# OpenDataPlane/odp

Hardware: AMD Instinct MI355X
Metric: Mpkts/s classified device-resident (higher is better)
Workload: dtype u8; 1 GPU; config3; packets_per_gpu=1000000, packets_total=1000000, rules=256, cos=33, frame_bytes=IMIX 60/566/1514 7:4:1, streams=1, rotate=4, parallelism=shard1

## Files before the change

odp_amd/csrc/mi_cls.hip:

```cpp
#include "mi_cls_dev.h"

#include "mi_cls_asm.h"
#include "mi_cls_spec.h"

#include <errno.h>
#include <unistd.h>

#include <algorithm>
#include <array>
#include <map>
#include <memory>
#include <mutex>
#include <set>
#include <string>
#include <thread>
#include <vector>

struct mi_cls_ctx {
	int device;
	uint32_t *d_dev;
	size_t dev_cap;
	int loaded;
	MiProgram prog;
	int wpb;
// ... 290 lines not shown
	const bool small = (long)hot_bytes <= (long)hot_max;
	const bool full4 = small && 4 * (st_of(4) + hot_bytes) <= LDS_CU;
	const bool small_batch = c->batch_hint != 0 &&
				 c->batch_hint < 2u * (uint32_t)c->num_cu * 16u * WAVE;
	int nw = 4;
	bool lt = full4;
	for (int w : { 16, 12, 8 })
		if (st_of(w) + hot_bytes <= LDS_CU) {
			nw = w;
			lt = true;
			break;
		}
	if ((nw == 8 || small_batch) && full4) {
		nw = 4;
		lt = true;
	}
	if (wpb_env == 4 || wpb_env == 8 || wpb_env == 12 || wpb_env == 16) {
		nw = wpb_env;
		lt = nw == 4 ? small && st_of(4) + hot_bytes <= LDS_CU : st_of(nw) + hot_bytes <= LDS_CU;
		if (nw != 4 && nw != 16 && !lt)
			nw = 16;
	}
	if (opt != 0 && nw != 4) {
		nw = 16;
		lt = st_of(16) + hot_bytes <= LDS_CU;
		if (!lt)
			nw = 4;
	}
	const size_t lds_block = st_of(nw) + (lt ? hot_bytes : 0);
	int per_cu = (int)(LDS_CU / lds_block);
	const int occ = MIN_WAVES_PER_EU;
	if (per_cu > occ * 4 / nw)
		per_cu = occ * 4 / nw;
	if (per_cu_env > 0)
		per_cu = per_cu_env;
	if (per_cu < 1)
		per_cu = 1;
	return Shape{ nw, lt, lt ? hot_bytes : 0, per_cu };
}


static void dump_spec(const std::string &src)
{
	const char *dp = getenv("MI_CLS_DUMP_SPEC");
	FILE *f = dp ? fopen(dp, "w") : nullptr;
	if (f) {
		fputs(src.c_str(), f);
		fclose(f);
	}
}

extern "C" int mi_cls_spec_compile(const void *tbl, size_t bytes, int nw)
{
	MiProgram p;
	const int rc = mi_asm_compile(tbl, bytes, mi_asm_knobs_from_env(), p);
	if (rc)
		return rc;
	if (nw != 4 && nw != 12 && nw != 16)
		return -EINVAL;
	if (p.spec_mode < 0 && p.plan.empty())
		return 1;
	std::string inst;
	const std::string src = mi_asm_spec_program(p, nw, true, false, inst);
	dump_spec(src);
	return mi_spec_compile_now(src, inst);
}

static bool spec_enabled(void)
{
	const char *e = getenv("MI_CLS_JIT");
	return !(e && e[0] == '0');
}

static void spec_setup(mi_cls_ctx_t *c)
{
	c->spec.reset();
	c->spec_fn = nullptr;
	const bool ck = c->opt != 0;
	const bool flat = c->prog.spec_mode >= 0;
	if ((!flat && c->prog.plan.empty()) || !spec_enabled())
		return;
	const Shape sh = pick_shape(c, c->opt);
	if (ck ? ((flat && !sh.lt) || (sh.nw != 4 && sh.nw != 16))
	       : flat ? (!sh.lt || (sh.nw != 4 && sh.nw != 12 && sh.nw != 16))
		      : (sh.nw != 4 && sh.nw != 8 && sh.nw != 12 && sh.nw != 16))
		return;
	std::string inst;
	const std::string src = mi_asm_spec_program(c->prog, sh.nw, flat ? true : sh.lt, ck, inst);
	dump_spec(src);
	c->spec = mi_spec_request(src, inst);
	c->spec_nw = sh.nw;
	c->spec_lt = sh.lt;
	c->spec_ck = ck;
}

static hipFunction_t spec_fn(mi_cls_ctx_t *c, bool wait)
{
	if (c->spec_fn || !c->spec)
		return c->spec_fn;
	hipFunction_t fn = nullptr;
	if (!mi_spec_function(*c->spec, c->device, wait, &fn))
		return nullptr;
	if (!fn)
		c->spec.reset();
	c->spec_fn = fn;
	return fn;
}


extern "C" int mi_cls_last_launch(const mi_cls_ctx_t *c, uint32_t *info, uint32_t n)
{
	if (!c || (!info && n))
		return -EINVAL;
	const uint32_t k = n < MI_CLS_LAUNCH_INFO_WORDS ? n : MI_CLS_LAUNCH_INFO_WORDS;
	memcpy(info, c->last, k * sizeof(uint32_t));
	return (int)k;
}

extern "C" int mi_cls_spec_wait(mi_cls_ctx_t *c)
{
	if (!c || !c->loaded)
		return -EINVAL;
	if (!c->spec)
		return 1;
	return spec_fn(c, true) ? 0 : 1;
}

extern "C" int mi_cls_classify(mi_cls_ctx_t *c, const uint8_t *pkts, const uint32_t *off,
			       const uint16_t *len, uint32_t n, mi_cls_result_t *out, void *stream)
{
	if (!c || !c->loaded)
		return -EINVAL;
	if (n == 0)
		return 0;
	if (!pkts || !off || !len || !out)
		return -EINVAL;
	if (((uintptr_t)out & 15u) != 0)
		return -EINVAL;
	HIP_OK(hipSetDevice(c->device));
	KArgs a;
	a.pkts = pkts;
	a.off = off;
	a.len = len;
	a.n = n;
	a.dev = c->d_dev;
	a.out = out;
	a.stats = c->stats_on ? c->d_stats : nullptr;
	a.opt = c->opt;
	a.hint = c->d_hint;
	a.seq = ++c->seq;
	if (a.seq == 0u)
		a.seq = c->seq = 2u;
	memcpy(a.stats_mask, c->stats_mask, sizeof(a.stats_mask));
	const Shape sh = pick_shape(c, c->opt);
	const int nw = sh.nw;
	const bool lt = sh.lt;
	const bool div = c->prog.tree;
	const uint32_t bthreads = (uint32_t)nw * WAVE;
	uint32_t tiles = (n + bthreads - 1) / bthreads;
	uint32_t max_grid = (uint32_t)c->num_cu * (uint32_t)sh.per_cu;
	uint32_t grid = tiles < max_grid ? tiles : max_grid;
	const size_t dyn = sh.dyn;
	hipStream_t st = (hipStream_t)stream;
	int lrc;
	uint32_t *last = c->last;
	last[0] = (uint32_t)nw;
	last[1] = lt;
	last[2] = 0;
	last[3] = 0;
	last[4] = 0;
	last[5] = c->opt != 0;
	last[6] = grid;
	const bool spec_ok = c->spec && c->spec_ck == (c->opt != 0) && c->spec_nw == nw &&
			     c->spec_lt == lt && spec_fn(c, false);
	if (c->opt != 0 && spec_ok) {
		last[2] = c->prog.flat_mode < 0 && div;
		last[3] = (uint32_t)(c->prog.flat_mode + 1);
		last[4] = 1;
		void *args[] = { &a };
		lrc = hipModuleLaunchKernel(c->spec_fn, grid, 1, 1, (unsigned)bthreads, 1, 1,
					    (unsigned)dyn, st, args, nullptr) == hipSuccess ? 0 : -EIO;
	} else if (c->opt != 0) {
		last[2] = div;
		lrc = mi_cls_launch_ck(nw, lt, div, grid, dyn, st, a);
	} else if (spec_ok) {
		last[2] = c->prog.flat_mode < 0 && div;
		last[3] = (uint32_t)(c->prog.flat_mode + 1);
		last[4] = 1;
		void *args[] = { &a };
		lrc = hipModuleLaunchKernel(c->spec_fn, grid, 1, 1, (unsigned)bthreads, 1, 1,
					    (unsigned)dyn, st, args, nullptr) == hipSuccess ? 0 : -EIO;
	} else if (c->prog.flat_mode >= 0 && c->prog.flat_mode != 1 && lt && (nw == 4 || nw == 12 || nw == 16)) {
		last[3] = (uint32_t)(c->prog.flat_mode + 1);
		lrc = mi_cls_launch_flat(nw, c->prog.flat_mode, grid, dyn, st, a);
	} else {
		last[2] = div;
		if (nw == 16)
			lrc = mi_cls_launch_k16(lt, div, grid, dyn, st, a);
		else if (nw == 12)
			lrc = mi_cls_launch_k12(lt, div, grid, dyn, st, a);
		else if (nw == 8)
			lrc = mi_cls_launch_k8(lt, div, grid, dyn, st, a);
		else
			lrc = mi_cls_launch_k4(lt, div, grid, dyn, st, a);
	}
	if (lrc)
		return lrc;
	if (hipGetLastError() != hipSuccess)
		return -EIO;
	return 0;
}


struct HostRange {
	size_t bytes;
	ptrdiff_t delta;
};
static std::mutex g_hreg_mu;
static std::map<uintptr_t, HostRange> g_hreg;

static const void *dev_view_slow(const void *p)
{
	hipPointerAttribute_t a;
	if (hipPointerGetAttributes(&a, p) != hipSuccess) {
		(void)hipGetLastError();
		return nullptr;
	}
	if (a.type != hipMemoryTypeHost || !a.devicePointer || !a.hostPointer)
		return nullptr;
	return (const uint8_t *)a.devicePointer + ((const uint8_t *)p - (const uint8_t *)a.hostPointer);
}

static const void *dev_view(const void *p)
{
	{
		std::lock_guard<std::mutex> lk(g_hreg_mu);
		auto it = g_hreg.upper_bound((uintptr_t)p);
		if (it != g_hreg.begin()) {
			--it;
			if ((uintptr_t)p - it->first < it->second.bytes)
				return (const uint8_t *)p + it->second.delta;
		}
	}
	return dev_view_slow(p);
}

template <typename T> static bool dev_views(T *&p)
{
	const void *d = dev_view(p);
	return d ? (p = (T *)d, true) : false;
}
template <typename T, typename... U> static bool dev_views(T *&p, U *&...more)
{
	return dev_views(p) && dev_views(more...);
}

static int no_ctx(void)
{
	return mi_cls_device_count() > 0 ? -EINVAL : -ENODEV;
}

static bool frames_inside(const uint32_t *off, const uint16_t *len, uint32_t n, size_t bytes)
{
	for (uint32_t i = 0; i < n; ++i)
		if ((size_t)off[i] + len[i] > bytes)
			return false;
	return true;
}

static bool frames_padded_inside(const uint32_t *off, const uint16_t *len, uint32_t n, size_t lim)
{
	for (uint32_t i = 0; i < n; ++i)
		if ((size_t)off[i] + (((size_t)len[i] + 15u) & ~(size_t)15u) > lim)
			return false;
	return true;
}

static int stage_bufs(mi_cls_ctx_t *c, size_t need, uint32_t n)
{
	if ((need > c->pk_cap || n > c->n_cap) && c->submitted)
		HIP_OK(hipStreamSynchronize(c->stream));
	if (need > c->pk_cap) {
		(void)hipFree(c->d_pk);
		c->d_pk = nullptr;
		size_t cap = need < (1u << 20) ? (1u << 20) : need + need / 2;
		if (hipMalloc((void **)&c->d_pk, cap) != hipSuccess)
			return c->pk_cap = 0, -ENOMEM;
		HIP_OK(hipMemset(c->d_pk, 0, cap));
		c->pk_cap = cap;
	}
	if (n > c->n_cap) {
		(void)hipFree(c->d_off);
		(void)hipFree(c->d_len);
		(void)hipFree(c->d_out);
		(void)hipHostFree(c->h_off);
		(void)hipHostFree(c->h_out);
		c->d_off = nullptr;
		c->d_len = nullptr;
		c->d_out = nullptr;
		c->h_off = nullptr;
		c->h_out = nullptr;
		uint32_t cap = n < 4096u ? 4096u : n + n / 2;
		if (hipMalloc((void **)&c->d_off, cap * sizeof(uint32_t)) != hipSuccess ||
		    hipMalloc((void **)&c->d_len, cap * sizeof(uint16_t)) != hipSuccess ||
		    hipMalloc((void **)&c->d_out, cap * sizeof(mi_cls_result_t)) != hipSuccess ||
		    hipHostMalloc((void **)&c->h_off, cap * sizeof(uint32_t), hipHostMallocDefault) != hipSuccess ||
// ... 1120 lines not shown
```

odp_amd/csrc/mi_cls_dev.h:

```cpp
#pragma once
#ifndef __HIPCC_RTC__
#include <hip/hip_runtime.h>
#include <errno.h>
#include <stdio.h>
#include <stdlib.h>
#include <string.h>
#endif
#include <stdint.h>

#include "mi_cls.h"
#include "mi_cls_prog.h"

#include <type_traits>

#define WAVE 64
#define WIN 96
#define WROWS (WIN / 4 + 1)
#define RS 66
#define NPIECE (WIN / 16)
#define MIN_WAVES_PER_EU 4
#define LOAD_AUX 2
#define MAX_STATS_COS 256

#define E_SNAP 1u
// ... 212 lines not shown
	}
	if ((err & E_IP) && (((f & F_IPV4) && (opt & OPT_DROP_V4)) ||
			     ((f & F_IPV6) && (opt & OPT_DROP_V6)))) {
		r.l4 = 0xFFFFu;
		r.flags = f;
		r.err = err;
		r.ret = -1;
		return r;
	}

	int ret = 0;
	f |= F_L4;
	switch (ip_proto) {
	case 1u:
	case 58u:
		f |= F_ICMP;
		break;
	case 4u:
		break;
	case 6u:
		f |= F_TCP;
		if (!non_first) {
			if (off + 20u > len)
				ret = -1;
			else if ((rb(k, off + 12) >> 4) < 5u)
				err |= E_TCP;
			if ((err & E_TCP) && (opt & OPT_DROP_TCP))
				ret = -1;
		}
		break;
	case 17u:
		f |= F_UDP;
		if (!non_first) {
			if (off + 8u > len) {
				ret = -1;
			} else {
				uint32_t ports = r32(k, off);
				uint32_t ulen = be16(k, off + 4);
				if (ulen < 8u) {
					err |= E_UDP;
					if (opt & OPT_DROP_UDP)
						ret = -1;
				} else {
					if ((opt & OPT_UDP_CK) && !(f & F_IPFRAG) && r16(k, off + 6) == 0u) {
						f |= F_L4CK_DONE;
						err |= (f & F_IPV4) ? 0u : E_L4CK;
						r.udp_zero = 1;
					}
					if ((ports >> 16) == 0x9411u  && ulen > 4u &&
					    r32(k, off + 8) != 0u)
						f |= F_IPSEC;
				}
			}
		}
		break;
	case 51u:
		f |= F_IPSEC | F_AH;
		break;
	case 50u:
		f |= F_IPSEC | F_ESP;
		break;
	case 132u:
		f |= F_SCTP;
		if (!non_first) {
			if (off + 12u > len)
				ret = -1;
			else if (((len - r.l4) & 0xffffu) < 12u)
				err |= E_SCTP;
			if ((err & E_SCTP) && (opt & OPT_DROP_SCTP))
				ret = -1;
		}
		break;
	case 59u:
		f |= F_NO_NEXT;
		break;
	default:
		f &= ~F_L4;
		break;
	}
	r.flags = f;
	r.err = err;
	r.ret = ret < 0 ? -1 : (err != 0 ? 1 : 0);
	return r;
}

#define OOB_OFF 0xFFFFFE00u

#define CRC_ZN 256
#define CRC_S128 1024u
#define CRC_S256 2048u
#define CRC_Z 3072u
#define CRC_YINV (CRC_Z + CRC_ZN)
#define CRC_Y1 (CRC_YINV + 65u)
#define CRC_WORDS (CRC_Y1 + 64u)
__host__ __device__ constexpr uint32_t crc_mulmod_c(uint32_t a, uint32_t b)
{
	uint32_t p = 0;
	for (int i = 31; i >= 0; --i) {
		p ^= ((a >> i) & 1u) ? b : 0u;
		b = (b >> 1) ^ ((b & 1u) ? 0x82F63B78u : 0u);
	}
	return p;
}
struct Crc32cTab {
	uint32_t t[4][256];
	uint32_t s128[4][256];
	uint32_t s256[4][256];
	uint32_t z[CRC_ZN];
	uint32_t yinv[65];
	uint32_t y1[64];
	constexpr Crc32cTab() : t(), s128(), s256(), z(), yinv(), y1()
	{
		for (uint32_t i = 0; i < 256; ++i) {
			uint32_t c = i;
			for (int b = 0; b < 8; ++b)
				c = (c & 1u) ? (c >> 1) ^ 0x82F63B78u : (c >> 1);
			t[0][i] = c;
		}
		for (int k = 1; k < 4; ++k)
			for (uint32_t i = 0; i < 256; ++i)
				t[k][i] = (t[k - 1][i] >> 8) ^ t[0][t[k - 1][i] & 0xffu];
		for (int k = 0; k < 4; ++k)
			for (uint32_t i = 0; i < 256; ++i) {
				uint32_t r = i << (8 * k);
				for (int j = 0; j < 32; ++j) {
					if (j == 16)
						s128[k][i] = r;
					r = t[0][r & 0xffu] ^ (r >> 8);
				}
				s256[k][i] = r;
			}
		uint32_t r = 0x80000000u;
		for (uint32_t m = 0; m < CRC_ZN; ++m) {
			z[m] = r;
			for (int i = 0; i < 16; ++i)
				r = t[3][r & 0xffu] ^ t[2][(r >> 8) & 0xffu] ^ t[1][(r >> 16) & 0xffu] ^
				    t[0][r >> 24];
		}
		uint32_t xi8 = 0x80000000u;
		for (int i = 0; i < 8; ++i)
			xi8 = crc_mulmod_c(xi8, (0x82F63B78u << 1) | 1u);
		r = 0x80000000u;
		for (uint32_t i = 0; i < 65; ++i) {
			yinv[i] = r;
			r = crc_mulmod_c(r, xi8);
		}
		r = 0xFFFFFFFFu;
		for (uint32_t i = 0; i < 64; ++i) {
			y1[i] = r;
			r = t[0][r & 0xffu] ^ (r >> 8);
		}
	}
};
static __constant__ Crc32cTab c_crc32c;

__device__ __forceinline__ uint32_t crc32c_u8(const uint32_t *tab, uint32_t crc, uint32_t b)
{
	return tab[(crc ^ b) & 0xffu] ^ (crc >> 8);
}

__device__ __forceinline__ uint32_t crc32c_u32(const uint32_t *tab, uint32_t crc, uint32_t w)
{
	const uint32_t c = crc ^ w;
	return tab[768u + (c & 0xffu)] ^ tab[512u + ((c >> 8) & 0xffu)] ^
	       tab[256u + ((c >> 16) & 0xffu)] ^ tab[c >> 24];
}

__device__ __forceinline__ uint32_t lane_get(uint32_t v, uint32_t src)
{
	return (uint32_t)__builtin_amdgcn_ds_bpermute((int)(src << 2), (int)v);
}

__device__ __forceinline__ uint32_t wave_scan_add(uint32_t v, uint32_t lane)
{
	v += (uint32_t)__builtin_amdgcn_update_dpp(0, (int)v, 0x111, 0xf, 0xf, true);
	v += (uint32_t)__builtin_amdgcn_update_dpp(0, (int)v, 0x112, 0xf, 0xf, true);
	v += (uint32_t)__builtin_amdgcn_update_dpp(0, (int)v, 0x114, 0xf, 0xf, true);
	v += (uint32_t)__builtin_amdgcn_update_dpp(0, (int)v, 0x118, 0xf, 0xf, true);
	const uint32_t r0 = (uint32_t)__builtin_amdgcn_readlane((int)v, 15);
	const uint32_t r1 = (uint32_t)__builtin_amdgcn_readlane((int)v, 31);
	const uint32_t r2 = (uint32_t)__builtin_amdgcn_readlane((int)v, 47);
	const uint32_t row = lane >> 4;
	return v + (row >= 1u ? r0 : 0u) + (row >= 2u ? r1 : 0u) + (row >= 3u ? r2 : 0u);
}

#define CK_HALVES 1
__device__ __forceinline__ uint32_t ck_sum_wave(__amdgpu_buffer_rsrc_t rs, uint32_t base,
						uint32_t prm, uint32_t cnt, uint32_t lane)
{
	const uint32_t incl = wave_scan_add(cnt, lane);
	const uint32_t first = incl - cnt;
	const uint32_t total = (uint32_t)__builtin_amdgcn_readlane((int)incl, WAVE - 1);
	uint32_t acc = 0;
	for (uint32_t B = 0; B < total; B += CK_HALVES * WAVE) {
		uint32_t r[CK_HALVES];
		{
			uint32_t ob[CK_HALVES];
			int32_t lb[CK_HALVES], hb[CK_HALVES];
			bool live[CK_HALVES];
#pragma unroll
			for (uint32_t h = 0; h < CK_HALVES; ++h) {
				const uint32_t g = B + WAVE * h + lane;
				uint32_t lo = 0;
#pragma unroll
				for (uint32_t st = WAVE / 2; st >= 1; st >>= 1) {
					const uint32_t c = lo + st;
					lo = lane_get(first, c) <= g ? c : lo;
				}
				const uint32_t q = g - lane_get(first, lo);
				const uint32_t pr = lane_get(prm, lo);
				ob[h] = lane_get(base, lo) + 64u * q;
				live[h] = g < total;
				lb[h] = (int32_t)(pr & 63u) - (int32_t)(64u * q);
				hb[h] = (int32_t)(pr >> 6) - (int32_t)(64u * q);
			}
			u32x4 v[CK_HALVES][4];
			uint32_t xh[CK_HALVES], xt[CK_HALVES];
			__builtin_amdgcn_s_setprio(3);
#pragma unroll
			for (uint32_t h = 0; h < CK_HALVES; ++h) {
#pragma unroll
				for (int32_t k = 0; k < 4; ++k)
					v[h][k] = __builtin_amdgcn_raw_buffer_load_b128(
						rs, (live[h] && 16 * k < hb[h] && 16 * k + 16 > lb[h]) ? ob[h] + 16u * k
													: OOB_OFF, 0, 0);
				const bool ph = live[h] && lb[h] > 0 && (lb[h] & 3) != 0;
				const bool pt = live[h] && hb[h] < 64 && (hb[h] & 3) != 0;
				xh[h] = __builtin_amdgcn_raw_buffer_load_b32(
					rs, ph ? ob[h] + (uint32_t)(lb[h] & ~3) : OOB_OFF, 0, 0);
				xt[h] = __builtin_amdgcn_raw_buffer_load_b32(
					rs, pt ? ob[h] + (uint32_t)(hb[h] & ~3) : OOB_OFF, 0, 0);
			}
			__builtin_amdgcn_s_setprio(0);
#pragma unroll
			for (uint32_t h = 0; h < CK_HALVES; ++h) {
				uint64_t sm = (uint64_t)(xh[h] >> 16) +
					      (xt[h] & ((1u << (8u * ((uint32_t)hb[h] & 3u))) - 1u));
				const uint32_t lo4 = (uint32_t)max(lb[h], 0);
				const int32_t sp = hb[h] - 4 - max(lb[h], 0);
#pragma unroll
				for (uint32_t d = 0; d < 16; ++d) {
					const bool in = live[h] && sp >= 0 && (4u * d - lo4) <= (uint32_t)sp;
					sm += in ? v[h][d >> 2][d & 3u] : 0u;
				}
				r[h] = (uint32_t)(sm & 0xffffu) + (uint32_t)(sm >> 16);
			}
		}
		uint32_t P[CK_HALVES], T = 0;
#pragma unroll
		for (uint32_t h = 0; h < CK_HALVES; ++h) {
			P[h] = wave_scan_add(r[h], lane) + T;
			T = (uint32_t)__builtin_amdgcn_readlane((int)P[h], WAVE - 1);
		}
		const uint32_t a = first > B ? first - B : 0u;
		const uint32_t e = min(incl > B ? incl - B : 0u, (uint32_t)(CK_HALVES * WAVE));
		const uint32_t ie = e > 0u ? e - 1u : 0u, ia = a > 0u ? a - 1u : 0u;
		uint32_t pe = 0, pa = 0;
#pragma unroll
		for (uint32_t h = 0; h < CK_HALVES; ++h) {
			const uint32_t xe = lane_get(P[h], ie & (WAVE - 1u));
			const uint32_t xa = lane_get(P[h], ia & (WAVE - 1u));
			pe = ie / WAVE == h ? xe : pe;
			pa = ia / WAVE == h ? xa : pa;
		}
		acc += (e > a) ? pe - (a > 0u ? pa : 0u) : 0u;
	}
	return acc;
}

#define CK_AHEAD 4
__device__ __forceinline__ uint32_t sctp_crc(const Pkt &k, __amdgpu_buffer_rsrc_t rs, uint32_t boff,
					     uint32_t l4, const uint32_t *tab)
{
	const uint32_t len = k.len, sh = l4 & 3u, j0 = l4 >> 2, n4 = (len - l4) >> 2;
	uint32_t crc = 0xffffffffu, prev = 0u;
	const uint32_t jend = j0 + n4;
	const uint32_t q0 = (j0 >> 2) << 2;
	u32x4 nx[CK_AHEAD];
#pragma unroll
	for (uint32_t i = 0; i < CK_AHEAD; ++i) {
		const uint32_t qi = q0 + 4u * i;
		nx[i] = __builtin_amdgcn_raw_buffer_load_b128(rs, (qi <= jend && 4u * qi < len)
								      ? boff + 4u * qi : OOB_OFF, 0, 0);
	}
	for (uint32_t q = q0; q <= jend; q += 4u) {
		const u32x4 v = nx[0];
#pragma unroll
		for (uint32_t i = 0; i + 1 < CK_AHEAD; ++i)
			nx[i] = nx[i + 1];
		{
			const uint32_t qn = q + 4u * CK_AHEAD;
			nx[CK_AHEAD - 1] = __builtin_amdgcn_raw_buffer_load_b128(
				rs, (qn <= jend && 4u * qn < len) ? boff + 4u * qn : OOB_OFF, 0, 0);
		}
#pragma unroll
		for (uint32_t t = 0; t < 4; ++t) {
			const uint32_t lo = q + t - 1u;
			const uint32_t w = __builtin_amdgcn_alignbyte(v[t], prev, sh);
			const bool in = q + t >= 1u && lo >= j0 && lo < jend;
			crc = in ? crc32c_u32(tab, crc, lo - j0 == 2u ? 0u : w) : crc;
			prev = v[t];
		}
	}
	for (uint32_t o = l4 + 4u * n4; o < len; ++o)
		crc = crc32c_u8(tab, crc, rb(k, o));
	return ~crc;
}
// ... 889 lines not shown
		const uint32_t val = bv_probe(H, key, act && present, nk, hb(4), hb(5), hb(6), hb(7));
		const uint32_t rw = val != 0u ? (val == BV_EMPTY ? 0u : val) : hb(3);
		const bool h = act && rw != 0u;
		nxt = h ? (rw & 0xffu) : nxt;
		nleaf = h ? ((rw >> 8) & 1u) : nleaf;
		nmark = h ? (rw >> 16) : nmark;
		hit = h ? 1u : hit;
		return;
	}
	uint32_t first;
	if constexpr (FM == FM_CHAIN) {
		first = chain_first<typename SpecOf<D>::type>(H, blk.h, act, k, p, x);
	} else if constexpr (CHAIN && FM < 0 && std::is_same<D, DescU>::value) {
		first = BV_NONE;
		DescU cur = blk;
		DescV ch = hb;
		for (;;) {
			first = min(first, bv_first<-1, true>(cur, ch, H, act, k, p, x));
			const uint32_t nx = ch(0) >> 8;
			if (nx == 0u)
				break;
			cur = DescU{ blk.h + nx, blk.h };
			ch = cur.hdr();
		}
	} else {
		first = bv_first<FM, CHAIN>(blk, hb, H, act, k, p, x, cos);
	}
	const bool h = act && first != BV_NONE;
	const uint32_t rw2 = H[res + (h ? first : 0u)];
	nxt = h ? (rw2 & 0xffu) : nxt;
	nleaf = h ? ((rw2 >> 8) & 1u) : nleaf;
	nmark = h ? (rw2 >> 16) : nmark;
	hit = h ? 1u : hit;
}

template <typename...> struct mi_void { typedef void type; };
template <typename S, typename = void> struct plan_n {
	static constexpr uint32_t v = 0;
};
template <typename S> struct plan_n<S, typename mi_void<decltype(S::nplan)>::type> {
	static constexpr uint32_t v = S::nplan;
};

template <uint32_t V> struct mi_uconst {
	static constexpr uint32_t value = V;
};
template <uint32_t N, uint32_t I = 0, typename F>
__device__ __forceinline__ void static_for(F &f)
{
	if constexpr (I < N) {
		f(mi_uconst<I>{});
		static_for<N, I + 1>(f);
	}
}

template <typename S, uint32_t I, uint32_t C>
__device__ __forceinline__ DescV plan_rec()
{
	DescV d;
#pragma unroll
	for (uint32_t i = 0; i < 16; ++i)
		d.v[i] = S::grec[I][C][i];
	return d;
}

template <typename S, uint32_t I, typename T>
__device__ __forceinline__ void plan_eval(T H, bool bvl, uint32_t cs, const Pkt &k, const Parsed &p,
					  const Fields &x, uint32_t &hit, uint32_t &nxt, uint32_t &nmark,
					  uint32_t &nleaf)
{
	constexpr const uint32_t *ji = S::ginfo[I];
	uint32_t rw;
	bool hv;
	if constexpr (ji[0] == 0u) {
		const DescV cr = plan_rec<S, I, 0>();
		uint32_t key[4], nk = cr(1);
		const bool present = bv_key(cr, k, p, x, key);
		joint_key(ji[14], cs, key, nk);
		const uint32_t val = bv_probe(H, key, bvl && present, nk, ji[9], ji[10], ji[11], ji[12]);
		const uint32_t miss = H[ji[13] + cs];
		rw = val != 0u ? (val == BV_EMPTY ? 0u : val) : miss;
		hv = rw != 0u;
	} else {
		uint32_t acc = H[ji[2] + cs];
		auto cls = [&](auto ic) {
			constexpr uint32_t kc = decltype(ic)::value;
			if constexpr (kc < ji[1]) {
				constexpr const uint32_t *ci = ji + 8u + 8u * kc;
				const DescV cr = plan_rec<S, I, kc>();
				uint32_t key[4], nk = cr(1);
				const bool present = bv_key(cr, k, p, x, key);
				joint_key(ci[6], cs, key, nk);
				const uint32_t val = bv_probe(H, key, bvl && present, nk, ci[1], ci[2], ci[3], ci[4]);
				acc &= val != 0u ? val : H[ci[5] + cs];
			}
		};
		static_for<BV_MAX_CLS>(cls);
		const uint32_t res = H[ji[3] + cs];
		rw = H[res + (acc != 0u ? (uint32_t)__builtin_ctz(acc) : 0u)];
		hv = acc != 0u;
	}
	const bool h = bvl && hv;
	nxt = h ? (rw & 0xffu) : nxt;
	nleaf = h ? ((rw >> 8) & 1u) : nleaf;
	nmark = h ? (rw >> 16) : nmark;
	hit = h ? 1u : hit;
}

__device__ __forceinline__ void linear_scan(cword_t prog, uint32_t rec0, uint32_t nr, bool grp,
					    const Pkt &k, const Parsed &p, const Fields &x,
					    uint32_t &done, uint32_t &nxt, uint32_t &nmark)
{
	for (uint32_t r = 0; r < nr; ++r) {
		const bool cand = grp && done == 0u;
		if (__ballot(cand) == 0ull)
			break;
		const uint32_t base = (rec0 + r) * REC_WORDS;
		const uint32_t w0 = prog[base];
		const uint32_t w1 = prog[base + 1];
		const uint32_t n_in = w0 & 0xfu, n_ext = (w0 >> 8) & 0xfu;
		bool ok = cand;
		uint32_t q = base + 2;
		for (uint32_t t = 0; t < n_in; ++t) {
			if (__ballot(ok) == 0ull)
				break;
			ok = term_ok(prog, q, k, p, x) && ok;
		}
		if (n_ext && __ballot(ok) != 0ull) {
			q = w1 >> 8;
			for (uint32_t t = 0; t < n_ext; ++t) {
				if (__ballot(ok) == 0ull)
					break;
				ok = term_ok(prog, q, k, p, x) && ok;
			}
		}
		nxt = ok ? (w1 & 0xffu) : nxt;
		nmark = ok ? (w0 >> 16) : nmark;
		done = ok ? 1u : done;
	}
}

struct KArgs {
	const uint8_t *pkts;
	const uint32_t *off;
	const uint16_t *len;
	uint32_t n;
	const uint32_t *dev;
	mi_cls_result_t *out;
	unsigned long long *stats;
	uint32_t stats_mask[8];
	uint32_t opt;
	uint32_t *hint;
	uint32_t seq;
};

__device__ __forceinline__ bool stats_bit(const KArgs &a, uint32_t c)
{
	return c < MAX_STATS_COS && ((a.stats_mask[c >> 5] >> (c & 31u)) & 1u);
}

static_assert(NPIECE == 6, "WIN is 96");
#define NB (NPIECE - 4)

__device__ __forceinline__ bool load_window(__amdgpu_buffer_rsrc_t rs, uint32_t off, uint32_t len,
					    uint32_t lane, u32x4 d[NPIECE], bool want_hi, uint32_t &win)
{
	const uint32_t q = lane & 3u, pp = lane >> 2;
#pragma unroll
	for (uint32_t r = 0; r < 4; ++r) {
		const int src = (int)((16u * r + pp) << 2);
		const uint32_t o = (uint32_t)__builtin_amdgcn_ds_bpermute(src, (int)off);
		const uint32_t L = (uint32_t)__builtin_amdgcn_ds_bpermute(src, (int)len);
		const uint32_t vo = 16u * q < L ? o + 16u * q : OOB_OFF;
		d[r] = __builtin_amdgcn_raw_buffer_load_b128(rs, vo, 0, LOAD_AUX);
	}
	const bool any_long = __ballot(len > 64u) != 0ull;
	const bool hi = any_long && want_hi;
	win = (any_long && !hi) ? 64u : (uint32_t)WIN;
	if (hi) {
		const uint32_t qb = lane % NB, pb = lane / NB;
#pragma unroll
		for (uint32_t r = 0; r < NB; ++r) {
			const int src = (int)(((64u / NB) * r + pb) << 2);
			const uint32_t o = (uint32_t)__builtin_amdgcn_ds_bpermute(src, (int)off);
			const uint32_t L = (uint32_t)__builtin_amdgcn_ds_bpermute(src, (int)len);
			const uint32_t c = 16u * (4u + qb);
			const uint32_t vo = c < L ? o + c : OOB_OFF;
			d[4 + r] = __builtin_amdgcn_raw_buffer_load_b128(rs, vo, 0, LOAD_AUX);
		}
	}
	return hi;
}

__device__ __forceinline__ void store_window(uint32_t *W, uint32_t lane, const u32x4 d[NPIECE],
					     bool hi, bool &hi_rows)
{
	const uint32_t q = lane & 3u, pp = lane >> 2;
#pragma unroll
	for (uint32_t r = 0; r < 4; ++r) {
		const uint32_t base = 4u * q * RS + 16u * r + pp;
#pragma unroll
		for (uint32_t i = 0; i < 4; ++i)
			W[base + i * RS] = d[r][i];
	}
	if (hi) {
		const uint32_t qb = lane % NB, pb = lane / NB;
#pragma unroll
		for (uint32_t r = 0; r < NB; ++r) {
			const uint32_t base = 4u * (4u + qb) * RS + (64u / NB) * r + pb;
#pragma unroll
			for (uint32_t i = 0; i < 4; ++i)
				W[base + i * RS] = d[4 + r][i];
		}
	} else if (hi_rows) {
#pragma unroll
		for (uint32_t row = 16; row < WIN / 4; ++row)
			W[row * RS + lane] = 0u;
	}
	hi_rows = hi;
}

__device__ __forceinline__ void zero_tail(uint32_t *W, uint32_t lane, uint32_t len)
{
	const uint32_t pad = (WIN / 4) * RS + lane;
	const uint32_t dw = len >> 2, b = len & 3u;
	const bool part = b != 0u && len < WIN;
	uint8_t *W8 = (uint8_t *)W;
	const uint32_t pb = (dw * RS + lane) * 4u;
	W8[(part && (b & 1u)) ? pb + b : pad * 4u + 1u] = 0;
	*(uint16_t *)(W8 + ((part && b <= 2u) ? pb + 2u : pad * 4u + 2u)) = 0;
	const uint32_t r0 = (len + 3u) >> 2;
	W[min(r0, (uint32_t)(WIN / 4)) * RS + lane] = 0u;
	W[min(r0 + 1u, (uint32_t)(WIN / 4)) * RS + lane] = 0u;
	W[min(r0 + 2u, (uint32_t)(WIN / 4)) * RS + lane] = 0u;
}

template <typename T> __device__ __forceinline__ uint32_t ld_desc(const T *p)
{
	return (uint32_t)*p;
}

__device__ __forceinline__ void store_rec(mi_cls_result_t *dst, uint4 r)
{
	u32x4 v = { r.x, r.y, r.z, r.w };
	__builtin_nontemporal_store(v, (u32x4 *)dst);
}

__device__ __forceinline__ void wave_lds_sync()
{
	__builtin_amdgcn_fence(__ATOMIC_RELEASE, "wavefront");
	__builtin_amdgcn_wave_barrier();
	__builtin_amdgcn_fence(__ATOMIC_ACQUIRE, "wavefront");
}

extern __shared__ __attribute__((aligned(16))) uint32_t s_dyn[];

constexpr int waves_per_eu(int nw)
{
	return nw == 4 ? MIN_WAVES_PER_EU : nw / 4;
}

template <bool LT, bool DIV, int NW, int FM = -1, bool CK = false, typename SPEC = void>
__global__ __launch_bounds__(NW * WAVE, waves_per_eu(NW)) void mi_cls_kernel(KArgs a)
{
	__shared__ uint32_t s_win[NW * RS * WROWS];
	__shared__ uint32_t s_cnt[MAX_STATS_COS];
	__shared__ uint32_t s_l4[256];
	__shared__ uint32_t s_next;
	__shared__ uint32_t s_crc[CK ? CRC_WORDS : 1];

	const uint32_t lane = threadIdx.x & (WAVE - 1);
	const uint32_t wave = threadIdx.x >> 6;
	uint32_t *W = s_win + wave * RS * WROWS;

	const cword_t dev = (cword_t)a.dev;
	const int32_t def_cos = (int32_t)dev[DH_DEFAULT];
	const int32_t err_cos = (int32_t)dev[DH_ERROR];
	const uint32_t def_valid = dev[DH_DEFAULT_VALID];
	const uint32_t max_hops = dev[DH_MAX_HOPS];
	const uint32_t hot_off = dev[DH_HOT_OFF];
	const cword_t hc = dev + hot_off;
	const cword_t prog = dev + dev[DH_PROG_OFF];
	const cword_t dce = hc + COS_WORDS * (uint32_t)max(def_cos, 0);
	const uint32_t d_nr = def_cos >= 0 ? dce[C_NR] : 0u;
	const uint32_t d_bv = DIV ? dce[C_BV] & C_BV_OFF : dce[C_BV] & 0x7fffffffu, d_rec0 = dce[C_REC0];
	const uint32_t j_off = DIV ? dev[DH_JOINT] : 0u;
	const bool stats_on = a.stats != nullptr;
	typedef typename std::conditional<LT, lword_t, gword_t>::type hot_t;
	hot_t H;
	const uint32_t nt = (a.n + WAVE - 1) / WAVE;
	const uint32_t G = gridDim.x;
	auto tile_of = [&](uint32_t j) -> uint32_t {
		const uint32_t t = blockIdx.x + G * j;
		return t < nt ? t : 0xFFFFFFFFu;
	};
	uint32_t tile = tile_of(wave), nx = tile_of(NW + wave), nn = 0xFFFFFFFFu;
	uint32_t d_off = 0, d_len = 0, n_off = 0, n_len = 0;
	{
		const uint32_t p0 = tile * WAVE + lane, p1 = nx * WAVE + lane;
		if (tile < nt && p0 < a.n) {
			d_off = ld_desc(a.off + p0);
			d_len = ld_desc(a.len + p0);
		}
		if (nx < nt && p1 < a.n) {
			n_off = ld_desc(a.off + p1);
			n_len = ld_desc(a.len + p1);
		}
	}
	const __amdgpu_buffer_rsrc_t rs = __builtin_amdgcn_make_buffer_rsrc(
		(void *)a.pkts, (short)0, (int)OOB_OFF, 0x00020000);
	u32x4 d[NPIECE];
	bool d_hi, hi_rows = true;
	bool want_hi = a.hint == nullptr || *(const uint32_t *)a.hint + 1u == a.seq;
	constexpr bool PLH = DIV && !CK;
	if constexpr (PLH)
		want_hi = false;
	bool saw_hi = false;
	uint32_t d_win = WIN, my_win = WIN;
	const uint32_t p_l3end = dev[DH_L3END], p_l4end = dev[DH_L4END], p_frend = dev[DH_FREND];
	if (tile < nt)
		d_hi = load_window(rs, d_off, d_len, lane, d, want_hi, d_win);
	if constexpr (LT) {
		const uint32_t hq = (dev[DH_HOT_WORDS] + 3u) >> 2;
		typedef const __attribute__((address_space(1))) u32x4 *gvec_t;
		const gvec_t src = (gvec_t)(a.dev + hot_off);
		u32x4 *dst = (u32x4 *)s_dyn;
		for (uint32_t i = threadIdx.x; i < hq; i += NW * WAVE)
			dst[i] = src[i];
		H = (lword_t)s_dyn;
	} else {
		H = (gword_t)(a.dev + hot_off);
	}

	if (stats_on) {
		for (uint32_t i = threadIdx.x; i < MAX_STATS_COS; i += NW * WAVE)
			s_cnt[i] = 0;
	}
	for (uint32_t i = threadIdx.x; i < 256u; i += NW * WAVE)
		s_l4[i] = c_l4tab.v[i];
	if constexpr (CK) {
		const uint32_t *cw = reinterpret_cast<const uint32_t *>(&c_crc32c);
		for (uint32_t i = threadIdx.x; i < CRC_WORDS; i += NW * WAVE)
			s_crc[i] = cw[i];
	}
	for (uint32_t r = WIN / 4; r < WROWS; ++r)
		W[r * RS + lane] = 0u;
	if (threadIdx.x == 0)
		s_next = 0u;
	__syncthreads();

	uint4 prev_rec = make_uint4(0, 0, 0, 0);
	uint32_t prev_pi = 0;
	bool prev_valid = false;
	for (; tile < nt; tile = nx, nx = nn) {
		const uint32_t pi = tile * WAVE + lane;
		const bool valid = pi < a.n;
		const uint32_t my_off = d_off, my_len = d_len;
		my_win = d_win;

		wave_lds_sync();
		store_window(W, lane, d, d_hi, hi_rows);
		zero_tail(W, lane, my_len);
		if (prev_valid)
			store_rec(a.out + prev_pi, prev_rec);
		prev_valid = false;

		auto prefetch = [&]() {
			d_off = n_off;
			d_len = n_len;
			uint32_t k = 0;
			if (nx < nt && lane == 0)
				k = atomicAdd(&s_next, 1u);
			k = (uint32_t)__builtin_amdgcn_readfirstlane((int)k);
			nn = nx < nt ? tile_of(2u * NW + k) : 0xFFFFFFFFu;
			const uint32_t p2 = nn * WAVE + lane;
			n_off = 0;
			n_len = 0;
			if (nn < nt && p2 < a.n) {
				n_off = ld_desc(a.off + p2);
				n_len = ld_desc(a.len + p2);
			}
			if (nx < nt)
				d_hi = load_window(rs, d_off, d_len, lane, d, want_hi, d_win);
		};
		auto prefetch_pri = [&]() {
			if constexpr (CK) {
				prefetch();
			} else {
				const bool pri = __ballot(n_len > 64u) != 0ull;
				if (pri)
					__builtin_amdgcn_s_setprio(3);
				prefetch();
				if (pri)
					__builtin_amdgcn_s_setprio(0);
			}
		};
		if constexpr (!PLH)
			prefetch_pri();
		wave_lds_sync();

		Pkt k;
		k.w = W + lane;
		k.g = a.pkts + my_off;
		k.len = my_len;
		k.win = PLH ? 64u : my_win;

		Parsed p;
		bool dfr = false;
		if constexpr (!CK) {
			bool slow;
			p = parse_fast(k, s_l4, slow, PLH ? (uint32_t)WIN : 0u, dfr);
			if (__ballot(slow) != 0ull) {
				if (slow)
					p = parse_packet(k, 0u);
			}
		} else {
			bool slow;
			p = parse_fast(k, s_l4, slow, 0u, dfr);
			p.udp_zero = 0;
			slow = slow || p.err != 0u;
			if (a.opt & OPT_IPV4_CK) {
				const bool v4 = !slow && (p.flags & F_IPV4) != 0u;
				if (__ballot(v4) != 0ull) {
					if (v4) {
						const uint32_t ihl = rb(k, p.l3) & 0xfu;
						uint64_t sum = 0;
						for (uint32_t i = 0; i < ihl; ++i)
							sum += r32(k, p.l3 + 4u * i);
						if (ck_finalize(sum) != 0xffffu)
							slow = true;
						else
							p.flags |= F_L3CK_DONE;
					}
				}
			}
			if (a.opt & OPT_UDP_CK) {
				const bool u = !slow && (p.flags & F_UDP) != 0u && !(p.flags & F_IPFRAG) &&
					       p.ret == 0;
				if (__ballot(u) != 0ull) {
					if (u && r16(k, p.l4 + 6u) == 0u)
						slow = true;
				}
			}
			if (__ballot(slow) != 0ull) {
				if (slow)
					p = parse_packet(k, a.opt);
			}
			if (a.opt & OPT_L4_CK)
				l4_chksum(k, p, a.opt, rs, my_off, lane, valid, s_crc);
		}
		Fields x = fields_of(k, p);
		uint32_t need;
		{
			const uint32_t l4h = (p.flags & F_TCP) ? 13u : ((p.flags & F_UDP) ? 6u : 0u);
			need = p_frend;
			need = max(need, p.l3 != 0xFFFFu ? p.l3 + max(p_l3end, (p.flags & F_IPV6) ? 40u : 20u) : 0u);
			need = max(need, p.l4 != 0xFFFFu ? p.l4 + max(p_l4end, l4h) : 0u);
		}
		u32x4 hv0 = { 0u, 0u, 0u, 0u }, hv1 = { 0u, 0u, 0u, 0u };
		bool hneed = false, any_h = false;
		if constexpr (PLH) {
			hneed = valid && my_len > 64u && (need > 64u || dfr);
			any_h = __ballot(hneed) != 0ull;
			if (any_h) {
				hv0 = __builtin_amdgcn_raw_buffer_load_b128(rs, hneed ? my_off + 64u : OOB_OFF, 0,
									     LOAD_AUX);
				hv1 = __builtin_amdgcn_raw_buffer_load_b128(
					rs, hneed && my_len > 80u ? my_off + 80u : OOB_OFF, 0, LOAD_AUX);
			}
			prefetch_pri();
		} else {
			want_hi = __ballot(valid && my_len > 64u && need > 64u) != 0ull;
			saw_hi = saw_hi || want_hi;
		}
		auto far_in = [&]() {
			if constexpr (PLH) {
				if (any_h) {
					if (hneed) {
#pragma unroll
						for (uint32_t i = 0; i < 4; ++i) {
							W[(16u + i) * RS + lane] = hv0[i];
							W[(20u + i) * RS + lane] = hv1[i];
						}
						zero_tail(W, lane, my_len);
					}
					wave_lds_sync();
					k.win = hneed ? (uint32_t)WIN : 64u;
					x.k.win = k.win;
					if (__ballot(dfr) != 0ull) {
						uint32_t e4, f4, nd;
						const bool tcp = dfr && (p.flags & F_TCP) != 0u && p.l4 + 20u <= my_len;
						const bool udp = dfr && (p.flags & F_UDP) != 0u && p.l4 + 8u <= my_len;
						l4_bytes(k, p.l4, tcp, udp, e4, f4, nd);
						if (dfr) {
							p.err |= e4;
							p.flags |= f4;
// ... 333 lines not shown
```

Baseline: 42310 Mpkts/s.

## Pass program header by kernel args and batch LDS table preloads in registers

The program header words move into the kernel argument struct, so the per-block scalar loads of header fields from device memory are skipped. The hot table, CRC table and L4 table are now fetched with batched 128-bit buffer loads issued up front into registers, then written to LDS, instead of serial load-store loops. The first packet window load is moved after these stores. This aims to cut block prologue latency at the cost of more registers for the preload batch and a larger kernel argument block.

```diff
diff --git a/odp_amd/csrc/mi_cls.hip b/odp_amd/csrc/mi_cls.hip
--- a/odp_amd/csrc/mi_cls.hip
+++ b/odp_amd/csrc/mi_cls.hip
@@ -466,6 +466,7 @@
 	if (a.seq == 0u)
 		a.seq = c->seq = 2u;
 	memcpy(a.stats_mask, c->stats_mask, sizeof(a.stats_mask));
+	memcpy(a.hdr, c->prog.w.data(), sizeof(a.hdr));
 	const Shape sh = pick_shape(c, c->opt);
 	const int nw = sh.nw;
 	const bool lt = sh.lt;
diff --git a/odp_amd/csrc/mi_cls_dev.h b/odp_amd/csrc/mi_cls_dev.h
--- a/odp_amd/csrc/mi_cls_dev.h
+++ b/odp_amd/csrc/mi_cls_dev.h
@@ -388,7 +388,7 @@
 		}
 	}
 };
-static __constant__ Crc32cTab c_crc32c;
+static __constant__ __attribute__((aligned(16))) Crc32cTab c_crc32c;
 
 __device__ __forceinline__ uint32_t crc32c_u8(const uint32_t *tab, uint32_t crc, uint32_t b)
 {
@@ -1584,6 +1584,7 @@
 	uint32_t opt;
 	uint32_t *hint;
 	uint32_t seq;
+	uint32_t hdr[DH_WORDS];
 };
 
 __device__ __forceinline__ bool stats_bit(const KArgs &a, uint32_t c)
@@ -1699,24 +1700,54 @@
 	__shared__ uint32_t s_cnt[MAX_STATS_COS];
 	__shared__ uint32_t s_l4[256];
 	__shared__ uint32_t s_next;
-	__shared__ uint32_t s_crc[CK ? CRC_WORDS : 1];
+	__shared__ __attribute__((aligned(CK ? 16 : 4))) uint32_t s_crc[CK ? CRC_WORDS : 1];
 
 	const uint32_t lane = threadIdx.x & (WAVE - 1);
 	const uint32_t wave = threadIdx.x >> 6;
 	uint32_t *W = s_win + wave * RS * WROWS;
 
 	const cword_t dev = (cword_t)a.dev;
-	const int32_t def_cos = (int32_t)dev[DH_DEFAULT];
-	const int32_t err_cos = (int32_t)dev[DH_ERROR];
-	const uint32_t def_valid = dev[DH_DEFAULT_VALID];
-	const uint32_t max_hops = dev[DH_MAX_HOPS];
-	const uint32_t hot_off = dev[DH_HOT_OFF];
+	const int32_t def_cos = (int32_t)a.hdr[DH_DEFAULT];
+	const int32_t err_cos = (int32_t)a.hdr[DH_ERROR];
+	const uint32_t def_valid = a.hdr[DH_DEFAULT_VALID];
+	const uint32_t max_hops = a.hdr[DH_MAX_HOPS];
+	const uint32_t hot_off = a.hdr[DH_HOT_OFF];
+	constexpr uint32_t NT = NW * WAVE;
+	constexpr uint32_t SETUP_HOT =
+		NW == 4 ? 5u : (160u * 1024u - (uint32_t)sizeof(s_win)) / 16u / NT + 1u;
+	static_assert(SETUP_HOT <= 14u, "the batch lives in registers");
+	const uint32_t hq = LT ? (a.hdr[DH_HOT_WORDS] + 3u) >> 2 : 0u;
+	const __amdgpu_buffer_rsrc_t hot_rs = __builtin_amdgcn_make_buffer_rsrc(
+		(void *)(a.dev + hot_off), (short)0, (int)(hq * 16u), 0x00020000);
+	u32x4 hot_p[LT ? SETUP_HOT : 1];
+	if constexpr (LT) {
+#pragma unroll
+		for (uint32_t j = 0; j < SETUP_HOT; ++j)
+			hot_p[j] = __builtin_amdgcn_raw_buffer_load_b128(hot_rs, (threadIdx.x + j * NT) * 16u, 0, 0);
+	}
+	constexpr uint32_t CRC_Q = CRC_WORDS / 4u;
+	constexpr uint32_t SETUP_CRC = CK ? (CRC_Q + NT - 1u) / NT : 1u;
+	static_assert(CRC_Q * 4u + 1u == CRC_WORDS, "one word past the 16-B pieces");
+	u32x4 crc_p[SETUP_CRC];
+	uint32_t crc_last = 0;
+	if constexpr (CK) {
+		const __amdgpu_buffer_rsrc_t crc_rs = __builtin_amdgcn_make_buffer_rsrc(
+			(void *)&c_crc32c, (short)0, (int)(CRC_Q * 16u), 0x00020000);
+#pragma unroll
+		for (uint32_t j = 0; j < SETUP_CRC; ++j)
+			crc_p[j] = __builtin_amdgcn_raw_buffer_load_b128(crc_rs, (threadIdx.x + j * NT) * 16u, 0, 0);
+		crc_last = reinterpret_cast<const uint32_t *>(&c_crc32c)[CRC_WORDS - 1u];
+	}
+	const __amdgpu_buffer_rsrc_t l4_rs = __builtin_amdgcn_make_buffer_rsrc(
+		(void *)&c_l4tab, (short)0, (int)sizeof(L4Tab), 0x00020000);
+	static_assert(NT >= 256u, "a thread per protocol number");
+	const uint32_t l4_p = __builtin_amdgcn_raw_buffer_load_b32(l4_rs, threadIdx.x * 4u, 0, 0);
 	const cword_t hc = dev + hot_off;
-	const cword_t prog = dev + dev[DH_PROG_OFF];
+	const cword_t prog = dev + a.hdr[DH_PROG_OFF];
 	const cword_t dce = hc + COS_WORDS * (uint32_t)max(def_cos, 0);
 	const uint32_t d_nr = def_cos >= 0 ? dce[C_NR] : 0u;
 	const uint32_t d_bv = DIV ? dce[C_BV] & C_BV_OFF : dce[C_BV] & 0x7fffffffu, d_rec0 = dce[C_REC0];
-	const uint32_t j_off = DIV ? dev[DH_JOINT] : 0u;
+	const uint32_t j_off = DIV ? a.hdr[DH_JOINT] : 0u;
 	const bool stats_on = a.stats != nullptr;
 	typedef typename std::conditional<LT, lword_t, gword_t>::type hot_t;
 	hot_t H;
@@ -1749,31 +1780,40 @@
 		want_hi = false;
 	bool saw_hi = false;
 	uint32_t d_win = WIN, my_win = WIN;
-	const uint32_t p_l3end = dev[DH_L3END], p_l4end = dev[DH_L4END], p_frend = dev[DH_FREND];
-	if (tile < nt)
-		d_hi = load_window(rs, d_off, d_len, lane, d, want_hi, d_win);
+	const uint32_t p_l3end = a.hdr[DH_L3END], p_l4end = a.hdr[DH_L4END], p_frend = a.hdr[DH_FREND];
 	if constexpr (LT) {
-		const uint32_t hq = (dev[DH_HOT_WORDS] + 3u) >> 2;
-		typedef const __attribute__((address_space(1))) u32x4 *gvec_t;
-		const gvec_t src = (gvec_t)(a.dev + hot_off);
 		u32x4 *dst = (u32x4 *)s_dyn;
-		for (uint32_t i = threadIdx.x; i < hq; i += NW * WAVE)
-			dst[i] = src[i];
+#pragma unroll
+		for (uint32_t j = 0; j < SETUP_HOT; ++j) {
+			const uint32_t i = threadIdx.x + j * NT;
+			if (i < hq)
+				dst[i] = hot_p[j];
+		}
+		for (uint32_t i = threadIdx.x + SETUP_HOT * NT; i < hq; i += NT)
+			dst[i] = __builtin_amdgcn_raw_buffer_load_b128(hot_rs, i * 16u, 0, 0);
 		H = (lword_t)s_dyn;
 	} else {
 		H = (gword_t)(a.dev + hot_off);
 	}
+	if constexpr (CK) {
+		u32x4 *dst = (u32x4 *)s_crc;
+#pragma unroll
+		for (uint32_t j = 0; j < SETUP_CRC; ++j) {
+			const uint32_t i = threadIdx.x + j * NT;
+			if (i < CRC_Q)
+				dst[i] = crc_p[j];
+		}
+		if (threadIdx.x == NT - 1u)
+			s_crc[CRC_WORDS - 1u] = crc_last;
+	}
+	if (threadIdx.x < 256u)
+		s_l4[threadIdx.x] = l4_p;
+	if (tile < nt)
+		d_hi = load_window(rs, d_off, d_len, lane, d, want_hi, d_win);
 
 	if (stats_on) {
 		for (uint32_t i = threadIdx.x; i < MAX_STATS_COS; i += NW * WAVE)
 			s_cnt[i] = 0;
-	}
-	for (uint32_t i = threadIdx.x; i < 256u; i += NW * WAVE)
-		s_l4[i] = c_l4tab.v[i];
-	if constexpr (CK) {
-		const uint32_t *cw = reinterpret_cast<const uint32_t *>(&c_crc32c);
-		for (uint32_t i = threadIdx.x; i < CRC_WORDS; i += NW * WAVE)
-			s_crc[i] = cw[i];
 	}
 	for (uint32_t r = WIN / 4; r < WROWS; ++r)
 		W[r * RS + lane] = 0u;
```

Result: faster. 43700 Mpkts/s (median of 6 runs) (+3.3%).
